# index-tts/index-tts

Measured on NVIDIA H100. Metric: speech_tokens_per_s, higher is better.
Workload: dtype bf16 GPT (bf16 weights/activations, fp32 accumulate, fp32 residual stream = the reference's use_bf16 autocast) + tail on wgmma with fp16 operands (.f16: DiT / WaveNet / BigVGAN-resblock GEMMs and the DiT flash attention; fp32 accumulate, fp32 softmax, fp32 residual streams and pointwise math) and tf

## Files before the change

index-tts_b200/csrc/gemm_tc.cu:

```cuda
#include "ops.h"
#include "ptx.cuh"
#include <cuda.h>
#include <cudaTypedefs.h>
#include <map>
#include <mutex>
#include <tuple>
#include <cstdlib>

namespace {

constexpr int BM = 128;
constexpr int BKB = 128;
constexpr int GEMM_THREADS = 160;

__device__ __forceinline__ float apply_act_tc(float v, int act) {
  switch (act) {
    case ACT_GELU_ERF: return 0.5f * v * (1.f + erff(v * 0.70710678118654752f));
    case ACT_SILU: return v / (1.f + __expf(-v));
    case ACT_MISH: {
      float sp = (v > 20.f) ? v : log1pf(__expf(v));
      return v * tanhf(sp);
    }
    case ACT_GELU_TANH: {
      float u = 0.7978845608028654f * (v + 0.044715f * v * v * v);
      return 0.5f * v * (1.f + tanhf(u));
    }
    case ACT_RELU: return v > 0.f ? v : 0.f;
    default: return v;
  }
}

struct TcParams {
  int M, N, K, taps, dil, pad, a_bcast, w_batched;
  int n_kchunks;
  const float* bias; int biasN; int act;
  const float* res; const float* rowscale; const float* colscale;
  int accum; float scale;
  float* out; long long out_batch_stride, out_off, out_valid; int ldo;
  int stages; int ring_bytes;
  int epi; __half* out16; const float* aux; int aux_stride;
};

constexpr int acc_tile_bytes(int BN) { return BM * (BN + 1) * 4; }

template <int BN, int EB>
__global__ void __launch_bounds__(GEMM_THREADS, 2)
gemm_tc_kernel(const __grid_constant__ CUtensorMap tmA, const __grid_constant__ CUtensorMap tmB,
               const TcParams p) {
  extern __shared__ __align__(1024) unsigned char smem_raw[];
  unsigned char* base = (unsigned char*)(((uintptr_t)smem_raw + 1023) & ~(uintptr_t)1023);
  constexpr int BK = BKB / EB;
  constexpr int A_BYTES = BM * BKB;
  constexpr int B_BYTES = BN * BKB;
  constexpr int STAGE_BYTES = A_BYTES + B_BYTES;
  constexpr int TP = BN + 1;
  uint64_t* full = (uint64_t*)(base + p.ring_bytes);
  uint64_t* empty = full + p.stages;

  const int warp = threadIdx.x >> 5, lane = threadIdx.x & 31;
  const int n0 = blockIdx.x * BN, m0 = blockIdx.y * BM, b = blockIdx.z;
  const int n_iters = p.taps * p.n_kchunks;

  if (threadIdx.x == 0) {
    for (int s = 0; s < p.stages; ++s) {
      ptx::mbar_init(&full[s], 1);
      ptx::mbar_init(&empty[s], 4);
    }
    ptx::fence_mbar_init();
  }
  __syncthreads();
  pdl_wait();
  pdl_trigger();

  if (warp == 4) {
    if (lane == 0) {
      ptx::prefetch_tensormap(&tmA);
      ptx::prefetch_tensormap(&tmB);
      for (int it = 0; it < n_iters; ++it) {
        const int s = it % p.stages;
        const uint32_t ph = (it / p.stages) & 1u;
        ptx::mbar_wait(&empty[s], ph ^ 1u);
        const int tap = it / p.n_kchunks, kc = it % p.n_kchunks;
        unsigned char* sa = base + (size_t)s * STAGE_BYTES;
        unsigned char* sb = sa + A_BYTES;
        ptx::mbar_arrive_expect_tx(&full[s], STAGE_BYTES);
        ptx::tma_load_3d(sa, &tmA, &full[s], kc * BK, m0 + tap * p.dil - p.pad, p.a_bcast ? 0 : b);
        ptx::tma_load_3d(sb, &tmB, &full[s], tap * p.K + kc * BK, n0, p.w_batched ? b : 0);
      }
    }
    return;
  }

  float acc0[BN / 2], acc1[BN / 2];
#pragma unroll
  for (int i = 0; i < BN / 2; ++i) { acc0[i] = 0.f; acc1[i] = 0.f; }
  for (int it = 0; it < n_iters; ++it) {
    const int s = it % p.stages;
    const uint32_t ph = (it / p.stages) & 1u;
    ptx::mbar_wait(&full[s], ph);
    const uint32_t sa = ptx::smem_u32(base + (size_t)s * STAGE_BYTES);
    const uint32_t sb = sa + A_BYTES;
    const uint64_t da = ptx::make_desc_sw128(sa), db = ptx::make_desc_sw128(sb);
    ptx::fence_regs(acc0);
    ptx::fence_regs(acc1);
    ptx::wgmma_fence();
#pragma unroll
    for (int k = 0; k < BKB / 32; ++k) {
      ptx::wgmma_ss<BN, EB>(acc0, da + (uint64_t)(2 * k), db + (uint64_t)(2 * k), 1u);
      ptx::wgmma_ss<BN, EB>(acc1, da + (uint64_t)(512 + 2 * k), db + (uint64_t)(2 * k), 1u);
    }
    ptx::wgmma_commit();
    ptx::wgmma_wait<1>();
    ptx::fence_regs(acc0);
    ptx::fence_regs(acc1);
    if (it > 0 && lane == 0) ptx::mbar_arrive(&empty[(it - 1) % p.stages]);
  }
  ptx::wgmma_wait<0>();
  ptx::fence_regs(acc0);
  ptx::fence_regs(acc1);

  ptx::named_bar_sync(1, 128);
  float* tile = (float*)base;
  {
    const int r0 = warp * 16 + (lane >> 2), c = 2 * (lane & 3);
#pragma unroll
    for (int j = 0; j < BN / 8; ++j) {
      float* t0 = tile + (size_t)r0 * TP + 8 * j + c;
      t0[0] = acc0[4 * j]; t0[1] = acc0[4 * j + 1];
      t0[8 * TP] = acc0[4 * j + 2]; t0[8 * TP + 1] = acc0[4 * j + 3];
      t0[64 * TP] = acc1[4 * j]; t0[64 * TP + 1] = acc1[4 * j + 1];
      t0[72 * TP] = acc1[4 * j + 2]; t0[72 * TP + 1] = acc1[4 * j + 3];
    }
  }
  ptx::named_bar_sync(1, 128);
  const int q = warp;
  const long long obs = p.out_batch_stride;
  const int biasN = p.biasN ? p.biasN : p.N;
  const int mrow0 = m0 + q * 32;
#pragma unroll 1
  for (int c0 = 0; c0 < BN; c0 += 32) {
    if (n0 + c0 >= p.N) break;
    const float* trow = tile + (size_t)(q * 32) * TP + c0;
    const int n = n0 + c0 + lane;
    if (p.epi != EPI_NONE) {
      const int row = mrow0 + lane;
      if (row < p.M) {
        const int nb = n0 + c0;
        float v[32];
#pragma unroll
        for (int j = 0; j < 32; ++j) v[j] = trow[lane * TP + j] + (p.bias ? __ldg(p.bias + nb + j) : 0.f);
        if (p.epi == EPI_ROPE) {
          const int HD = 64, Hh = p.aux_stride, HW = Hh * HD;
          const int which = nb / HW, hh = (nb % HW) / HD, d0 = nb % HD;
          __half* dst = p.out16 + (size_t)which * ((size_t)gridDim.z * Hh * p.M * HD) + (((size_t)b * Hh + hh) * (size_t)p.M + row) * HD + d0;
          uint32_t o[16];
          if (which < 2) {
            const float4* tab = (const float4*)(p.aux + ((size_t)row * (HD / 2) + (d0 >> 1)) * 2);
            const float sc = (which == 0) ? p.scale : 1.0f;
#pragma unroll
            for (int i = 0; i < 8; ++i) {
              const float4 t4 = __ldg(tab + i);
              const float a0 = v[4 * i], a1 = v[4 * i + 1], b0 = v[4 * i + 2], b1 = v[4 * i + 3];
              __half2 h0 = __floats2half2_rn((a0 * t4.x - a1 * t4.y) * sc, (a1 * t4.x + a0 * t4.y) * sc);
              __half2 h1 = __floats2half2_rn((b0 * t4.z - b1 * t4.w) * sc, (b1 * t4.z + b0 * t4.w) * sc);
              o[2 * i] = *(uint32_t*)&h0;
              o[2 * i + 1] = *(uint32_t*)&h1;
            }
          } else {
#pragma unroll
            for (int i = 0; i < 16; ++i) {
              __half2 h = __floats2half2_rn(v[2 * i], v[2 * i + 1]);
              o[i] = *(uint32_t*)&h;
            }
          }
#pragma unroll
          for (int i = 0; i < 4; ++i) ((uint4*)dst)[i] = make_uint4(o[4 * i], o[4 * i + 1], o[4 * i + 2], o[4 * i + 3]);
        } else {
          const int NH = p.N >> 1, j0 = nb >> 1;
          uint32_t o[8];
#pragma unroll
          for (int i = 0; i < 8; ++i) {
            float r0, r1;
            if (p.epi == EPI_SWIGLU) {
              r0 = __fdividef(v[4 * i], 1.f + __expf(-v[4 * i])) * v[4 * i + 1];
              r1 = __fdividef(v[4 * i + 2], 1.f + __expf(-v[4 * i + 2])) * v[4 * i + 3];
            } else {
              const float* ga = p.aux + (size_t)b * p.aux_stride + j0 + 2 * i;
              r0 = tanhf(v[4 * i] + __ldg(ga)) * __fdividef(1.f, 1.f + __expf(-(v[4 * i + 1] + __ldg(ga + NH))));
              r1 = tanhf(v[4 * i + 2] + __ldg(ga + 1)) * __fdividef(1.f, 1.f + __expf(-(v[4 * i + 3] + __ldg(ga + NH + 1))));
            }
            __half2 h = __floats2half2_rn(r0, r1);
            o[i] = *(uint32_t*)&h;
          }
          uint4* dst = (uint4*)(p.out16 + ((size_t)b * p.M + row) * NH + j0);
          dst[0] = make_uint4(o[0], o[1], o[2], o[3]);
          dst[1] = make_uint4(o[4], o[5], o[6], o[7]);
        }
      }
    } else if (n < p.N) {
      const float bv = p.bias ? __ldg(p.bias + (n % biasN)) : 0.f;
      const float cs = (p.colscale ? __ldg(p.colscale + n) : 1.f);
      const long long flat0 = p.out_off + (long long)mrow0 * p.ldo + n;
      const int rows = min(32, p.M - mrow0);
      const bool interior = rows == 32 && (p.out_off + (long long)mrow0 * p.ldo + n0 + c0) >= 0 &&
                            (p.out_off + (long long)(mrow0 + 31) * p.ldo + n0 + c0 + 31) < p.out_valid;
      float* op = p.out + (long long)b * obs + flat0;
      const float* rp = p.res ? p.res + (long long)b * obs + flat0 : nullptr;
      if (interior && p.act == ACT_NONE && !p.rowscale) {
        const float sc = p.scale;
        if (!rp && !p.accum) {
#pragma unroll 8
          for (int rr = 0; rr < 32; ++rr) op[(long long)rr * p.ldo] = (trow[rr * TP + lane] + bv) * cs * sc;
        } else {
          float addv[32];
#pragma unroll
          for (int rr = 0; rr < 32; ++rr) {
            float a = 0.f;
            if (rp) a = rp[(long long)rr * p.ldo];
            if (p.accum) a += op[(long long)rr * p.ldo];
            addv[rr] = a;
          }
#pragma unroll
          for (int rr = 0; rr < 32; ++rr)
            op[(long long)rr * p.ldo] = ((trow[rr * TP + lane] + bv) * cs + addv[rr]) * sc;
        }
      } else {
        for (int rr = 0; rr < rows; ++rr) {
          const long long flat = flat0 + (long long)rr * p.ldo;
          if (flat < 0 || flat >= p.out_valid) continue;
          float v = trow[rr * TP + lane] + bv;
          v = apply_act_tc(v, p.act) * cs;
          if (p.rowscale) v *= __ldg(p.rowscale + (long long)b * p.M + mrow0 + rr);
          if (rp) v += rp[(long long)rr * p.ldo];
          if (p.accum) v += op[(long long)rr * p.ldo];
          op[(long long)rr * p.ldo] = v * p.scale;
        }
      }
    }
  }
}

PFN_cuTensorMapEncodeTiled get_encode() {
  static PFN_cuTensorMapEncodeTiled fn = nullptr;
  if (!fn) {
    void* f = nullptr;
    cudaDriverEntryPointQueryResult qres;
    if (cudaGetDriverEntryPoint("cuTensorMapEncodeTiled", &f, cudaEnableDefault, &qres) != cudaSuccess || !f)
      throw IdxError(IDX_ERR_CUDA, "cuTensorMapEncodeTiled entry point not available");
    fn = (PFN_cuTensorMapEncodeTiled)f;
  }
  return fn;
}

using MapKey = std::tuple<const void*, long long, long long, long long, long long, int, int>;
std::map<MapKey, CUtensorMap>& map_cache() {
  static std::map<MapKey, CUtensorMap> c;
  return c;
}

CUtensorMap make_map(const void* ptr, int rank, const cuuint64_t* dims, const cuuint64_t* strides_bytes,
                     const cuuint32_t* box, bool half = false) {
  static const bool plain_f32 = getenv("IDX_TMA_F32") != nullptr;
  MapKey key(ptr, (long long)dims[0], (long long)dims[1], rank > 2 ? (long long)dims[2] : 0,
             (long long)strides_bytes[0] ^ ((rank > 2 ? (long long)strides_bytes[1] : 0) << 20), (int)box[1] | ((int)box[0] << 12), rank | (half ? 16 : 0));
  static std::mutex mu;
  std::lock_guard<std::mutex> lock(mu);
  auto& cache = map_cache();
  auto it = cache.find(key);
  if (it != cache.end()) return it->second;
  CUtensorMap m;
  cuuint32_t estr[3] = {1, 1, 1};
  CUresult r = get_encode()(&m, half ? CU_TENSOR_MAP_DATA_TYPE_FLOAT16 : (plain_f32 ? CU_TENSOR_MAP_DATA_TYPE_FLOAT32 : CU_TENSOR_MAP_DATA_TYPE_TFLOAT32),
                            (cuuint32_t)rank, const_cast<void*>(ptr), dims, strides_bytes, box, estr,
                            CU_TENSOR_MAP_INTERLEAVE_NONE, CU_TENSOR_MAP_SWIZZLE_128B,
                            CU_TENSOR_MAP_L2_PROMOTION_L2_128B, CU_TENSOR_MAP_FLOAT_OOB_FILL_NONE);
  if (r != CUDA_SUCCESS)
    throw IdxError(IDX_ERR_CUDA, "cuTensorMapEncodeTiled failed with code " + std::to_string((int)r));
  if (cache.size() > 20000) cache.clear();
  cache.emplace(key, m);
  return m;
}

template <int BN, int EB>
void launch_bn(idx_engine* e, const ConvGemm& g, const CUtensorMap& tmA, const CUtensorMap& tmB) {
  constexpr int BK = BKB / EB;
  TcParams p;
  p.M = g.M; p.N = g.N; p.K = g.K; p.taps = g.taps; p.dil = g.dil; p.pad = g.pad; p.a_bcast = g.a_bcast;
  p.w_batched = g.w_batch_stride != 0;
  p.n_kchunks = (g.K + BK - 1) / BK;
  p.bias = g.bias; p.biasN = g.biasN; p.act = g.act;
  p.res = g.res; p.rowscale = g.rowscale; p.colscale = g.colscale;
  p.accum = g.accum; p.scale = g.scale; p.out = g.out;
  p.ldo = g.ldo ? g.ldo : g.N;
  p.out_batch_stride = g.out_batch_stride ? g.out_batch_stride : (long long)g.M * g.N;
  p.out_off = g.out_off;
  p.out_valid = g.out_valid ? g.out_valid : (long long)g.M * p.ldo;
  p.epi = g.epi; p.out16 = g.out16; p.aux = g.aux; p.aux_stride = g.aux_stride;
  if (g.epi != EPI_NONE)
    IDX_CHECK(g.out16 && g.N % 32 == 0 && !g.res && !g.accum && g.act == ACT_NONE && (g.epi == EPI_SWIGLU || g.aux), IDX_ERR_ARG,
              "conv_gemm: bad fused-epilogue arguments");
  constexpr int STAGE = BM * BKB + BN * BKB;
  const int n_iters = p.taps * p.n_kchunks;
  static const int occ = getenv("IDX_GEMM_OCC") ? atoi(getenv("IDX_GEMM_OCC")) : 2;
  int stages = ((occ == 1 ? 208 : 104) * 1024) / STAGE;
  if (stages > 8) stages = 8;
  if (stages > n_iters) stages = n_iters < 2 ? 2 : n_iters;
  p.stages = stages;
  p.ring_bytes = ((stages * STAGE > acc_tile_bytes(BN) ? stages * STAGE : acc_tile_bytes(BN)) + 1023) & ~1023;
  const size_t smem = (size_t)p.ring_bytes + 1024 + 2 * stages * 8;
  const unsigned bit = (BN == 32 ? 1u : (BN == 64 ? 2u : 4u)) << (EB == 2 ? 8 : 0);
  if (!(e->attr_done & bit)) {
    IDX_CUDA(cudaFuncSetAttribute(gemm_tc_kernel<BN, EB>, cudaFuncAttributeMaxDynamicSharedMemorySize, 220 * 1024));
    e->attr_done |= bit;
  }
  dim3 grid((g.N + BN - 1) / BN, (g.M + BM - 1) / BM, g.B);
  launch_pdl(e, gemm_tc_kernel<BN, EB>, grid, dim3(GEMM_THREADS), smem, tmA, tmB, p);
  e->launches++;
}


constexpr int FA_Q = 128, FA_K = 128, FA_D = 64;
constexpr int FA_THREADS = 288;
__device__ __forceinline__ float ex2_approx(float x) {
  float y;
  asm("ex2.approx.ftz.f32 %0, %1;" : "=f"(y) : "f"(x));
  return y;
}
__device__ __forceinline__ uint32_t pack_half2(float lo, float hi) {
  __half2 h = __floats2half2_rn(lo, hi);
  return *(uint32_t*)&h;
}
struct FaParams {
  int T, H; float* out; __half* out16; const int4* tiles;
  const int* lens; const float* qe; int rel_l, rel_r;
};
template <int SEL>
__device__ __forceinline__ void fa_add_relkey(float (&S)[FA_K / 2], const float* qr, int r, int k0, int t4, int L, int R) {
  if (k0 + FA_K - 1 - r <= -L || k0 - r >= R) {
    const float c = qr[k0 - r >= R ? L + R : 0];
#pragma unroll
    for (int c8 = 0; c8 < FA_K / 8; ++c8) { S[4 * c8 + SEL] += c; S[4 * c8 + SEL + 1] += c; }
  } else {
#pragma unroll
    for (int c8 = 0; c8 < FA_K / 8; ++c8) {
      const int d = k0 + 8 * c8 + 2 * t4 - r;
      S[4 * c8 + SEL] += qr[min(max(d, -L), R) + L];
      S[4 * c8 + SEL + 1] += qr[min(max(d + 1, -L), R) + L];
    }
  }
}
constexpr int FA_QE = 80;
// ... 265 lines not shown
```

index-tts_b200/csrc/nn_ops.cu:

```cuda
#include "ops.h"
#include <cuda_bf16.h>
#include <cstdlib>

namespace {

__device__ __forceinline__ float warp_sum(float v) {
#pragma unroll
  for (int o = 16; o > 0; o >>= 1) v += __shfl_xor_sync(0xffffffffu, v, o);
  return v;
}

__device__ __forceinline__ void put(float* __restrict__ y, __half* __restrict__ y16, long long i, float v) {
  if (y) y[i] = v;
  if (y16) y16[i] = __float2half_rn(v);
}

template <int MODE>
__global__ void rownorm_kernel(const float* __restrict__ x, float* __restrict__ y, long long rows, int T,
                               int C, const float* __restrict__ w, const float* __restrict__ b, float eps,
                               const float* __restrict__ m0, const float* __restrict__ m1, int mod_stride,
                               __half* __restrict__ y16) {
  pdl_wait();
  const long long row = (long long)blockIdx.x * (blockDim.x >> 5) + (threadIdx.x >> 5);
  const int lane = threadIdx.x & 31;
// ... 90 lines not shown
  const int t = blockIdx.y;
  const int c = blockIdx.x * blockDim.x + threadIdx.x;
  const int id = ids[t];
  const bool ok = id >= 0 && id < nrows;
  if (!ok && c == 0) atomicCAS(bad, 0, t + 1);
  if (c < C) out[(long long)t * C + c] = ok ? table[(long long)id * C + c] : 0.f;
}

__global__ void swiglu_kernel(const float* __restrict__ ab, float* __restrict__ y, long long rows, int N, __half* __restrict__ y16) {
  pdl_wait();
  const long long i = (long long)blockIdx.x * blockDim.x + threadIdx.x;
  if (i >= rows * N) return;
  const long long r = i / N;
  const int c = (int)(i % N);
  const float a = ab[r * 2 * N + c], b = ab[r * 2 * N + N + c];
  put(y, y16, i, a / (1.f + expf(-a)) * b);
}

__global__ void wn_gate_kernel(const float* __restrict__ xin, const float* __restrict__ g, int g_stride,
                               float* __restrict__ y, int T, int N, __half* __restrict__ y16) {
  pdl_wait();
  const int bi = blockIdx.z;
  const long long i = (long long)blockIdx.x * blockDim.x + threadIdx.x;
  if (i >= (long long)T * N) return;
  const long long t = i / N;
  const int c = (int)(i % N);
  const float* xr = xin + ((long long)bi * T + t) * 2 * N;
  const float a = xr[c] + g[(long long)bi * g_stride + c];
  const float s = xr[N + c] + g[(long long)bi * g_stride + N + c];
  put(y, y16, ((long long)bi * T + t) * N + c, tanhf(a) * (1.f / (1.f + expf(-s))));
}

__global__ void copy_cols_kernel(const float* __restrict__ src, int lds, float* __restrict__ dst, int ldo,
                                 int col0, long long rows, int C, __half* __restrict__ dst16) {
  pdl_wait();
  const long long i = (long long)blockIdx.x * blockDim.x + threadIdx.x;
  if (i >= rows * C) return;
  const long long r = i / C;
  const int c = (int)(i % C);
  put(dst, dst16, r * ldo + col0 + c, src[r * lds + c]);
}
__global__ void bcast_cols_kernel(const float* __restrict__ vec, float* __restrict__ dst, int ldo, int col0,
                                  int T, int C) {
  const int bi = blockIdx.z;
  const long long i = (long long)blockIdx.x * blockDim.x + threadIdx.x;
  if (i >= (long long)T * C) return;
  const long long t = i / C;
  const int c = (int)(i % C);
  dst[((long long)bi * T + t) * ldo + col0 + c] = vec[(long long)bi * C + c];
}
__global__ void silu_kernel(float* x, long long n) {
  const long long i = (long long)blockIdx.x * blockDim.x + threadIdx.x;
  if (i < n) { const float v = x[i]; x[i] = v / (1.f + expf(-v)); }
}
__device__ __forceinline__ int reflect_src(int i, int T, int left, int right) {
  const int Tr = max(T, max(left, right) + 1);
  int t = i - left;
  if (t < 0) t = -t;
  if (t >= Tr) t = 2 * (Tr - 1) - t;
  return t < T ? t : -1;
}
__global__ void reflect_pad_kernel(const float* __restrict__ x, float* __restrict__ y, int T, int C, int left, int right,
                                   int Tout, __half* __restrict__ y16) {
  pdl_wait();
  const int bi = blockIdx.z;
  const int c = blockIdx.x * blockDim.x + threadIdx.x;
  if (c >= C) return;
  for (int i = blockIdx.y; i < Tout; i += gridDim.y) {
    const int t = reflect_src(i, T, left, right);
    put(y, y16, ((long long)bi * Tout + i) * C + c, t >= 0 ? x[((long long)bi * T + t) * C + c] : 0.f);
  }
}
__device__ __forceinline__ int segment_of(const int* __restrict__ off, int n, int r, int gap) {
  int lo = 0, hi = n - 1;
  while (lo < hi) {
    const int mid = (lo + hi + 1) >> 1;
    if (off[mid] + mid * gap <= r) lo = mid; else hi = mid - 1;
  }
  return lo;
}
__global__ void reflect_pad_seg_kernel(const float* __restrict__ x, __half* __restrict__ y16, int T, int C, int left, int gap,
                                       int Tout, const int* __restrict__ off, int n) {
  pdl_wait();
  const int bi = blockIdx.z;
  const int c = blockIdx.x * blockDim.x + threadIdx.x;
  if (c >= C) return;
  for (int i = blockIdx.y; i < Tout; i += gridDim.y) {
    const int u = segment_of(off, n, i, gap);
    const int t0 = off[u], Tu = off[u + 1] - t0;
    const int t = reflect_src(i - t0 - u * gap, Tu, left, gap - left);
    y16[((long long)bi * Tout + i) * C + c] = __float2half_rn(t >= 0 ? x[((long long)bi * T + t0 + t) * C + c] : 0.f);
  }
}
__global__ void compact_seg_kernel(const __half* __restrict__ x, __half* __restrict__ y, int T, int Mg, int C, int gap,
                                   const int* __restrict__ off, int n) {
  pdl_wait();
  const int bi = blockIdx.z;
  const int c = (blockIdx.x * blockDim.x + threadIdx.x) * 8;
  if (c >= C) return;
  for (int r = blockIdx.y; r < T; r += gridDim.y) {
    const int u = segment_of(off, n, r, 0);
    *(uint4*)(y + ((long long)bi * T + r) * C + c) = *(const uint4*)(x + ((long long)bi * Mg + r + u * gap) * C + c);
  }
}
__global__ void cfg_euler_rows_kernel(float* x, const float* vc, const float* vu, float dt, float rate, int T, int C,
                                      const unsigned char* __restrict__ zero_rows) {
  pdl_wait();
  const long long i = (long long)blockIdx.x * blockDim.x + threadIdx.x;
  if (i >= (long long)T * C) return;
  const int t = (int)(i / C);
  const float d = (1.0f + rate) * vc[i] - rate * vu[i];
  x[i] = zero_rows[t] ? 0.f : x[i] + dt * d;
}
// ... 598 lines not shown
```

index-tts_b200/csrc/ops.h:

```cpp
#pragma once
#include "engine.h"
#include <cuda_fp16.h>
#include <cstdlib>
#include <string>
#include <utility>
#include <vector>

enum { EPI_NONE = 0, EPI_SWIGLU = 1, EPI_WNGATE = 2, EPI_ROPE = 3 };
enum { ACT_NONE = 0, ACT_GELU_ERF = 1, ACT_SILU = 2, ACT_MISH = 3, ACT_GELU_TANH = 4, ACT_RELU = 5 };

struct ConvGemm {
  const float* A = nullptr;
  int B = 1, Tin = 0, K = 0;
  long long a_batch_stride = 0;
  int a_bcast = 0;
  int lda = 0;
  const float* W = nullptr;
  const float* Wk = nullptr;
  const __half* A16 = nullptr;
  const __half* Wk16 = nullptr;
  int epi = 0;
  __half* out16 = nullptr;
  const float* aux = nullptr;
  int aux_stride = 0;
  long long w_batch_stride = 0;
  int ldw = 0;
  int taps = 1, dil = 1, pad = 0, reflect = 0;
  int M = 0;
  int N = 0;
  const float* bias = nullptr;
  int biasN = 0;
  int act = ACT_NONE;
  const float* res = nullptr;
  const float* rowscale = nullptr;
  const float* colscale = nullptr;
  int accum = 0;
  float scale = 1.f;
  float* out = nullptr;
  long long out_batch_stride = 0;
  long long out_off = 0;
  long long out_valid = 0;
  int ldo = 0;
};

void conv_gemm(idx_engine* e, const ConvGemm& g);
inline int gemm_default_backend(const idx_engine* e) { return e->gemm_backend; }

void transpose_bct_to_btc(idx_engine* e, const float* in, float* out, int B, int C, int T);
void transpose_btc_to_bct(idx_engine* e, const float* in, float* out, int B, int T, int C);

#ifdef __CUDACC__
__device__ __forceinline__ void pdl_wait() { asm volatile("griddepcontrol.wait;" ::: "memory"); }
__device__ __forceinline__ void pdl_trigger() { asm volatile("griddepcontrol.launch_dependents;" ::: "memory"); }
template <typename... KArgs, typename... Args>
inline void launch_pdl(idx_engine* e, void (*kernel)(KArgs...), dim3 grid, dim3 block, size_t smem, Args&&... args) {
  static const bool off = getenv("IDX_PDL") && atoi(getenv("IDX_PDL")) == 0;
  cudaLaunchConfig_t cfg = {};
  cfg.gridDim = grid; cfg.blockDim = block; cfg.dynamicSmemBytes = smem; cfg.stream = e->stream;
  cudaLaunchAttribute attr[1];
  attr[0].id = cudaLaunchAttributeProgrammaticStreamSerialization;
  attr[0].val.programmaticStreamSerializationAllowed = 1;
  cfg.attrs = attr; cfg.numAttrs = off ? 0 : 1;
  IDX_CUDA(cudaLaunchKernelEx(&cfg, kernel, std::forward<Args>(args)...));
}
#endif

void layernorm(idx_engine* e, const float* x, float* y, int B, int T, int C, const float* w,
               const float* b, float eps, const float* scale, const float* shift, int mod_stride, __half* y16 = nullptr);
void rmsnorm_adaln(idx_engine* e, const float* x, float* y, int B, int T, int C, const float* nw,
                   const float* mw, const float* mb, int mod_stride, float eps, __half* y16 = nullptr);
void groupnorm1_mish(idx_engine* e, const float* x, float* y, int B, int T, int C, const float* w,
                     const float* b, float eps);
void dwconv1d(idx_engine* e, const float* x, float* y, int B, int T, int C, const float* w,
              const float* b, int k);
void nearest_interp(idx_engine* e, const float* x, float* y, int B, int Tin, int Tout, int C);
void embedding_rows(idx_engine* e, const float* table, const int* ids, float* out, int n, int C, int nrows);
void swiglu(idx_engine* e, const float* ab, float* y, long long rows, int N, __half* y16 = nullptr);
void wn_gate(idx_engine* e, const float* xin, const float* g, int g_stride, float* y, int B, int T, int N, __half* y16 = nullptr);
void copy_cols(idx_engine* e, const float* src, int lds, float* dst, int ldo, int col0, long long rows, int C, __half* dst16 = nullptr);
void bcast_cols(idx_engine* e, const float* vec, float* dst, int ldo, int col0, int B, int T, int C);
void silu_inplace(idx_engine* e, float* x, long long n);
void rope_table(idx_engine* e, float* tab, int T, int hd);
void attention_rope(idx_engine* e, const float* qkv, float* out, int B, int T, int H, const float* rope,
                    const int* lens, __half* out16 = nullptr);
void cfg_euler(idx_engine* e, float* x, const float* v_cond, const float* v_uncond, float dt, float rate,
               int T, int C, int P);
void fill_zero(idx_engine* e, float* x, long long n);
struct DebugOverrides {
  idx_engine* e;
  ~DebugOverrides() { e->force_backend = 0; e->force_tile_n = 0; }
};
void reflect_pad_rows(idx_engine* e, const float* x, float* y, int B, int T, int C, int left, int right, __half* y16 = nullptr);

struct PackedW {
  float* wsimt = nullptr;
  float* wk = nullptr;
  __half* wk16 = nullptr;
  const float* bias = nullptr;
  int N = 0, K = 0, taps = 1, dil = 1;
};
struct WeightPool {
  std::vector<void*> owned;
  float* alloc(size_t n);
  void release();
};
PackedW pack_linear(idx_engine* e, WeightPool& pool, const std::string& name, int row0 = 0, int rows = -1,
// ... 39 lines not shown
```

index-tts_b200/csrc/s2mel.cu:

```cuda
#include "stages.h"
#include <algorithm>
#include <cmath>
#include <cstring>

namespace {

__global__ void timestep_embed_kernel(const float* t, const float* freqs, float* out, int half) {
  const int k = blockIdx.x, i = threadIdx.x;
  if (i >= half) return;
  const float a = 1000.f * t[k] * freqs[i];
  out[(long long)k * 2 * half + i] = cosf(a);
  out[(long long)k * 2 * half + half + i] = sinf(a);
}

__global__ void gamma_residual_kernel(const float* y, const float* gamma, float* x, long long rows, int C) {
  const long long i = (long long)blockIdx.x * blockDim.x + threadIdx.x;
  if (i >= rows * C) return;
  x[i] += gamma[i % C] * y[i];
}

}

struct AdaLN {
  const float* norm_w = nullptr;
  int mod_off = 0;
};

struct S2melState {
  idx_s2mel_config cfg;
  idx_codec_config ccfg;
  bool has_s2mel = false, has_codec = false;
  WeightPool pool;
  int inter = 0;
  std::vector<PackedW> wqkv, wo, w13, w2, skip_in;
  std::vector<AdaLN> attn_norm, ffn_norm;
  AdaLN final_norm;
  PackedW mod_stack;
  PackedW cond_proj, merge_x, merge_rest, skip_linear, conv1, res_proj, fl_linear, conv2, fl_mod;
  PackedW te_mlp0, te_mlp2, te2_mlp0, te2_mlp2, wn_cond;
  const float *te_freqs = nullptr, *te2_freqs = nullptr;
  std::vector<PackedW> wn_in, wn_res, wn_skip;
  std::vector<__half*> w13_i16, wn_in_i16;
  std::vector<float*> wn_in_bias_i;
  int mod_width = 0;
  PackedW lr_in_proj, lr_out;
  std::vector<PackedW> lr_conv;
  std::vector<const float*> lr_gn_w, lr_gn_b;
  PackedW cd_out_proj, cd_embed, cd_head, cd_up;
  const float* cd_codebook = nullptr;
  const float *cd_norm_w = nullptr, *cd_norm_b = nullptr, *cd_fnorm_w = nullptr, *cd_fnorm_b = nullptr;
  struct CNX { const float *dw_w, *dw_b, *n_w, *n_b, *gamma; PackedW pw1, pw2; };
  std::vector<CNX> cnx;
  double ms_codec = 0, ms_lr = 0, ms_cfm = 0;
  cudaEvent_t ev0 = nullptr, ev1 = nullptr;
};

void s2mel_destroy(S2melState* s) {
  if (!s) return;
  s->pool.release();
  if (s->ev0) cudaEventDestroy(s->ev0);
  if (s->ev1) cudaEventDestroy(s->ev1);
  delete s;
}

static S2melState* state(idx_engine* e) {
  if (!e->s2mel) {
    e->s2mel = new S2melState();
    IDX_CUDA(cudaEventCreate(&e->s2mel->ev0));
    IDX_CUDA(cudaEventCreate(&e->s2mel->ev1));
  }
  return e->s2mel;
}

static PackedW pack_stacked(idx_engine* e, WeightPool& pool, const std::vector<std::string>& names, float** bias_out) {
  int K = -1, N = 0;
  for (auto& n : names) {
    const DevTensor& w = e->W(n + ".weight");
    IDX_CHECK(w.shape.size() >= 2, IDX_ERR_ARG, n + ": bad shape");
    if (K < 0) K = (int)w.shape[1];
    IDX_CHECK((int)w.shape[1] == K, IDX_ERR_ARG, n + ": K mismatch in stacked pack");
    N += (int)w.shape[0];
  }
  float* cat = nullptr;
  IDX_CUDA(cudaMalloc((void**)&cat, (size_t)N * K * 4));
  float* bias = pool.alloc(N);
  IDX_CUDA(cudaMemsetAsync(bias, 0, (size_t)N * 4, e->stream));
  int r = 0;
  for (auto& n : names) {
    const DevTensor& w = e->W(n + ".weight");
    const int rows = (int)w.shape[0];
    IDX_CUDA(cudaMemcpyAsync(cat + (size_t)r * K, w.d, (size_t)rows * K * 4, cudaMemcpyDeviceToDevice, e->stream));
    if (e->has(n + ".bias"))
      IDX_CUDA(cudaMemcpyAsync(bias + r, e->W(n + ".bias").d, (size_t)rows * 4, cudaMemcpyDeviceToDevice, e->stream));
    r += rows;
// ... 28 lines not shown
  s->attn_norm.clear(); s->ffn_norm.clear();
  for (int l = 0; l < Dn; ++l) {
    const std::string p = E + "transformer.layers." + std::to_string(l) + ".";
    s->wqkv.push_back(pack_linear(e, s->pool, p + "attention.wqkv"));
    s->wo.push_back(pack_linear(e, s->pool, p + "attention.wo"));
    s->w13.push_back(pack_stacked(e, s->pool, {p + "feed_forward.w1", p + "feed_forward.w3"}, nullptr));
    s->w13.back().bias = nullptr;
    s->w2.push_back(pack_linear(e, s->pool, p + "feed_forward.w2"));
    s->skip_in.push_back(pack_linear(e, s->pool, p + "skip_in_linear"));
    AdaLN a; a.norm_w = e->Wf(p + "attention_norm.norm.weight"); a.mod_off = (int)mods.size() * 2 * H;
    mods.push_back(p + "attention_norm.project_layer");
    AdaLN f; f.norm_w = e->Wf(p + "ffn_norm.norm.weight"); f.mod_off = (int)mods.size() * 2 * H;
    mods.push_back(p + "ffn_norm.project_layer");
    s->attn_norm.push_back(a);
    s->ffn_norm.push_back(f);
  }
  s->final_norm.norm_w = e->Wf(E + "transformer.norm.norm.weight");
  s->final_norm.mod_off = (int)mods.size() * 2 * H;
  mods.push_back(E + "transformer.norm.project_layer");
  s->mod_stack = pack_stacked(e, s->pool, mods, nullptr);
  s->mod_width = (int)mods.size() * 2 * H;
  s->cond_proj = pack_linear(e, s->pool, E + "cond_projection");
  {
    const DevTensor& w = e->W(E + "cond_x_merge_linear.weight");
    const int Kall = (int)w.shape[1];
    IDX_CHECK(Kall == H + 2 * C + cfg->style_dim, IDX_ERR_ARG, "cond_x_merge_linear shape");
    std::vector<float> h((size_t)H * Kall);
    IDX_CUDA(cudaMemcpy(h.data(), w.d, h.size() * 4, cudaMemcpyDeviceToHost));
    std::vector<float> hx((size_t)H * C), hr((size_t)H * (Kall - C));
    for (int r = 0; r < H; ++r) {
      memcpy(&hx[(size_t)r * C], &h[(size_t)r * Kall], (size_t)C * 4);
      memcpy(&hr[(size_t)r * (Kall - C)], &h[(size_t)r * Kall + C], (size_t)(Kall - C) * 4);
    }
    int64_t shx[2] = {H, C}, shr[2] = {H, Kall - C};
    IDX_CHECK(idx_load_weight(e, "__merge_x.weight", hx.data(), IDX_F32, 2, shx) == 0, IDX_ERR_ARG, e->err);
    IDX_CHECK(idx_load_weight(e, "__merge_rest.weight", hr.data(), IDX_F32, 2, shr) == 0, IDX_ERR_ARG, e->err);
    s->merge_x = pack_linear(e, s->pool, "__merge_x", 0, -1, false);
    s->merge_rest = pack_linear(e, s->pool, "__merge_rest", 0, -1, false);
    s->merge_rest.bias = e->Wf(E + "cond_x_merge_linear.bias");
  }
  s->skip_linear = pack_linear(e, s->pool, E + "skip_linear");
  s->conv1 = pack_linear(e, s->pool, E + "conv1");
  s->res_proj = pack_linear(e, s->pool, E + "res_projection");
  s->fl_linear = pack_linear(e, s->pool, E + "final_layer.linear");
  s->fl_mod = pack_linear(e, s->pool, E + "final_layer.adaLN_modulation.1");
  s->conv2 = pack_linear(e, s->pool, E + "conv2");
  s->te_mlp0 = pack_linear(e, s->pool, E + "t_embedder.mlp.0");
  s->te_mlp2 = pack_linear(e, s->pool, E + "t_embedder.mlp.2");
  s->te2_mlp0 = pack_linear(e, s->pool, E + "t_embedder2.mlp.0");
  s->te2_mlp2 = pack_linear(e, s->pool, E + "t_embedder2.mlp.2");
  s->te_freqs = e->Wf(E + "t_embedder.freqs");
  s->te2_freqs = e->Wf(E + "t_embedder2.freqs");
  s->wn_cond = pack_linear(e, s->pool, E + "wavenet.cond_layer.conv.conv");
  s->wn_in.clear(); s->wn_res.clear(); s->wn_skip.clear();
  for (int i = 0; i < NL; ++i) {
    const std::string wi = E + "wavenet.in_layers." + std::to_string(i) + ".conv.conv";
    const std::string wr = E + "wavenet.res_skip_layers." + std::to_string(i) + ".conv.conv";
    s->wn_in.push_back(pack_conv1d(e, s->pool, wi, 1));
    IDX_CHECK(s->wn_in.back().taps == cfg->wn_kernel, IDX_ERR_ARG, "wavenet kernel size");
    if (i < NL - 1) {
      s->wn_res.push_back(pack_linear(e, s->pool, wr, 0, WH));
      s->wn_skip.push_back(pack_linear(e, s->pool, wr, WH, WH));
    } else {
      s->wn_res.push_back(PackedW());
      s->wn_skip.push_back(pack_linear(e, s->pool, wr, 0, WH));
    }
  }
  const std::string R = "s2mel.length_regulator.";
  s->lr_in_proj = pack_linear(e, s->pool, R + "content_in_proj");
  s->lr_conv.clear(); s->lr_gn_w.clear(); s->lr_gn_b.clear();
  for (int i = 0; i < cfg->lr_convs; ++i) {
    s->lr_conv.push_back(pack_conv1d(e, s->pool, R + "model." + std::to_string(3 * i), 1));
    s->lr_gn_w.push_back(e->Wf(R + "model." + std::to_string(3 * i + 1) + ".weight"));
    s->lr_gn_b.push_back(e->Wf(R + "model." + std::to_string(3 * i + 1) + ".bias"));
  }
  s->lr_out = pack_linear(e, s->pool, R + "model." + std::to_string(3 * cfg->lr_convs));
  IDX_CUDA(cudaStreamSynchronize(e->stream));
  for (auto* v : {&s->wqkv, &s->wo, &s->w13, &s->w2, &s->skip_in, &s->wn_in, &s->wn_res, &s->wn_skip})
    for (auto& w : *v) pack_half(e, s->pool, w);
  for (auto* w : {&s->skip_linear, &s->conv1, &s->res_proj, &s->fl_linear, &s->conv2}) pack_half(e, s->pool, *w);
  s->w13_i16.clear(); s->wn_in_i16.clear(); s->wn_in_bias_i.clear();
  for (auto& w : s->w13) s->w13_i16.push_back(pack_half_interleaved(e, s->pool, w, nullptr));
  for (auto& w : s->wn_in) {
    float* bi = nullptr;
    s->wn_in_i16.push_back(pack_half_interleaved(e, s->pool, w, &bi));
    s->wn_in_bias_i.push_back(bi);
  }
  s->has_s2mel = true;
  IDX_API_END(e)
}

extern "C" int idx_codec_init(idx_engine* e, const idx_codec_config* cfg) {
  IDX_API_BEGIN
  IDX_CHECK(e && cfg, IDX_ERR_ARG, "null argument");
  IDX_CUDA(cudaSetDevice(e->device));
  S2melState* s = state(e);
  s->ccfg = *cfg;
  const std::string Q = "codec.quantizer.quantizers.0.", D = "codec.decoder.0.";
  s->cd_codebook = e->Wf(Q + "codebook.weight");
  s->cd_out_proj = pack_linear(e, s->pool, Q + "out_project");
  s->cd_embed = pack_conv1d(e, s->pool, D + "embed", 1);
  s->cd_norm_w = e->Wf(D + "norm.weight"); s->cd_norm_b = e->Wf(D + "norm.bias");
  s->cd_fnorm_w = e->Wf(D + "final_layer_norm.weight"); s->cd_fnorm_b = e->Wf(D + "final_layer_norm.bias");
  s->cnx.clear();
  for (int l = 0; l < cfg->vocos_num_layers; ++l) {
    const std::string p = D + "convnext." + std::to_string(l) + ".";
    S2melState::CNX c;
    c.dw_w = e->Wf(p + "dwconv.weight"); c.dw_b = e->Wf(p + "dwconv.bias");
    c.n_w = e->Wf(p + "norm.weight"); c.n_b = e->Wf(p + "norm.bias");
    c.gamma = e->Wf(p + "gamma");
    c.pw1 = pack_linear(e, s->pool, p + "pwconv1");
    c.pw2 = pack_linear(e, s->pool, p + "pwconv2");
    s->cnx.push_back(c);
  }
  s->cd_head = pack_linear(e, s->pool, "codec.decoder.1");
  s->cd_up = pack_conv1d(e, s->pool, "codec.up", 1);
  IDX_CUDA(cudaStreamSynchronize(e->stream));
  s->has_codec = true;
  IDX_API_END(e)
}

void codec_decode_dev(idx_engine* e, S2melState* s, const int* d_codes, int n, float* d_out) {
  const idx_codec_config& c = s->ccfg;
  const int Hs = c.hidden_size, Vd = c.vocos_dim, Vi = c.vocos_intermediate_dim;
  float* emb = e->arena.get<float>((size_t)n * c.codebook_dim);
  float* q = e->arena.get<float>((size_t)n * Hs);
  float* x = e->arena.get<float>((size_t)n * Vd);
  float* y = e->arena.get<float>((size_t)n * Vd);
  float* hbuf = e->arena.get<float>((size_t)n * Vi);
  float* up = e->arena.get<float>((size_t)2 * n * Hs);
  embedding_rows(e, s->cd_codebook, d_codes, emb, n, c.codebook_dim, c.codebook_size);
// ... 69 lines not shown
  for (int l = 0; l < Dn; ++l) {
    if (l > Dn / 2) {
      float* sk = skips[--nskip];
      copy_cols(e, h, H, hf ? nullptr : b.cat, 2 * H, 0, (long long)Bn * T, H, b.cat16);
      copy_cols(e, sk, H, hf ? nullptr : b.cat, 2 * H, H, (long long)Bn * T, H, b.cat16);
      float* hn = b.h[8 + (l & 1)];
      conv_gemm(e, G(s->skip_in[l], b.cat, b.cat16, Bn, T, hn));
      h = hn;
    }
    rmsnorm_adaln(e, h, hf ? nullptr : b.a, Bn, T, H, s->attn_norm[l].norm_w, mod + s->attn_norm[l].mod_off,
                  mod + s->attn_norm[l].mod_off + H, 0, 1e-5f, b.a16);
    if (hf && fused) {
      ConvGemm g = gemm_of16(s->wqkv[l], b.a16, Bn, T, nullptr);
      g.epi = EPI_ROPE; g.out16 = b.qkv16; g.aux = b.rope; g.aux_stride = nh;
      g.scale = flash_attention_q_scale();
      conv_gemm(e, g);
      const size_t one = (size_t)Bn * nh * T * 64;
      if (b.sg) flash_attention_wgmma_varlen(e, b.qkv16, b.qkv16 + one, b.qkv16 + 2 * one, nullptr, b.att16, Bn, nh, *b.sg);
      else flash_attention_split(e, b.qkv16, b.qkv16 + one, b.qkv16 + 2 * one, nullptr, b.att16, Bn, T, nh);
    } else {
      conv_gemm(e, G(s->wqkv[l], b.a, b.a16, Bn, T, b.qkv));
      attention_rope(e, b.qkv, hf ? nullptr : b.att, Bn, T, nh, b.rope, b.lens, b.att16);
    }
    float* hout = (l < Dn / 2) ? b.h[1 + l] : b.h[10 + (l & 1)];
    {
      ConvGemm g = G(s->wo[l], b.att, b.att16, Bn, T, hout);
      g.res = h;
      conv_gemm(e, g);
    }
    rmsnorm_adaln(e, hout, hf ? nullptr : b.a, Bn, T, H, s->ffn_norm[l].norm_w, mod + s->ffn_norm[l].mod_off,
                  mod + s->ffn_norm[l].mod_off + H, 0, 1e-5f, b.a16);
    if (hf && fused) {
      ConvGemm g = gemm_of16(s->w13[l], b.a16, Bn, T, nullptr);
      g.Wk16 = s->w13_i16[l]; g.bias = nullptr; g.epi = EPI_SWIGLU; g.out16 = b.ffh16;
      conv_gemm(e, g);
    } else {
      conv_gemm(e, G(s->w13[l], b.a, b.a16, Bn, T, b.ff));
      swiglu(e, b.ff, hf ? nullptr : b.qkv, (long long)Bn * T, s->inter, b.ffh16);
    }
    {
      ConvGemm g = G(s->w2[l], b.qkv, b.ffh16, Bn, T, hout);
      g.res = hout;
      conv_gemm(e, g);
    }
    h = hout;
    if (l < Dn / 2) skips[nskip++] = h;
  }
  rmsnorm_adaln(e, h, b.a, Bn, T, H, s->final_norm.norm_w, mod + s->final_norm.mod_off,
                mod + s->final_norm.mod_off + H, 0, 1e-5f);
  copy_cols(e, b.a, H, hf ? nullptr : b.cat, H + C, 0, (long long)Bn * T, H, b.cat16);
  for (int bi = 0; bi < Bn; ++bi)
    copy_cols(e, x_bcast ? x_t : x_t + (size_t)bi * T * C, C, hf ? nullptr : b.cat + (size_t)bi * T * (H + C), H + C, H, T, C,
              hf ? b.cat16 + (size_t)bi * T * (H + C) : nullptr);
  conv_gemm(e, G(s->skip_linear, b.cat, b.cat16, Bn, T, b.xres));
  if (hf) to_half(e, b.xres, b.xres16, (long long)Bn * T * H);
  conv_gemm(e, G(s->conv1, b.xres, b.xres16, Bn, T, b.wy));
  fill_zero(e, b.wout, (long long)Bn * T * WH);
  for (int i = 0; i < NL; ++i) {
    const int kk = s->wn_in[i].taps, pl = (kk - 1) - (kk - 1) / 2, pr = (kk - 1) / 2;
    if (b.sg) {
      const int gap = kk - 1, ng = b.sg->n();
      reflect_pad_segments(e, b.wy, b.wpad16, Bn, WH, pl, pr, *b.sg);
      ConvGemm gi = gemm_of16(s->wn_in[i], b.wpad16, Bn, T + ng * gap, nullptr);
      gi.pad = 0; gi.M = T + (ng - 1) * gap;
      gi.Wk16 = s->wn_in_i16[i]; gi.bias = s->wn_in_bias_i[i];
      gi.epi = EPI_WNGATE; gi.out16 = b.wacts16g; gi.aux = wncond + (size_t)i * 2 * WH; gi.aux_stride = 0;
      conv_gemm(e, gi);
      compact_segments16(e, b.wacts16g, b.wacts16, Bn, WH, gap, *b.sg);
    } else {
      reflect_pad_rows(e, b.wy, hf ? nullptr : b.wpad, Bn, T, WH, pl, pr, b.wpad16);
      ConvGemm gi = G(s->wn_in[i], b.wpad, b.wpad16, Bn, T + kk - 1, b.wxin);
      gi.pad = 0; gi.M = T;
      if (hf && fused) {
        gi.Wk16 = s->wn_in_i16[i]; gi.bias = s->wn_in_bias_i[i]; gi.out = nullptr;
        gi.epi = EPI_WNGATE; gi.out16 = b.wacts16; gi.aux = wncond + (size_t)i * 2 * WH; gi.aux_stride = 0;
        conv_gemm(e, gi);
      } else {
        conv_gemm(e, gi);
        wn_gate(e, b.wxin, wncond + (size_t)i * 2 * WH, 0, hf ? nullptr : b.wacts, Bn, T, WH, b.wacts16);
      }
    }
    if (i < NL - 1) {
      ConvGemm gr = G(s->wn_res[i], b.wacts, b.wacts16, Bn, T, b.wy);
      gr.res = b.wy;
      conv_gemm(e, gr);
    }
    ConvGemm gs = G(s->wn_skip[i], b.wacts, b.wacts16, Bn, T, b.wout);
    gs.accum = 1;
    conv_gemm(e, gs);
  }
  {
    ConvGemm g = G(s->res_proj, b.xres, b.xres16, Bn, T, b.wout);
    g.accum = 1;
    conv_gemm(e, g);
  }
  layernorm(e, b.wout, hf ? nullptr : b.z, Bn, T, WH, nullptr, nullptr, 1e-6f, flmod + WH, flmod, 0, b.z16);
  conv_gemm(e, G(s->fl_linear, b.z, b.z16, Bn, T, b.wy));
  if (hf) to_half(e, b.wy, b.wy16, (long long)Bn * T * WH);
  conv_gemm(e, G(s->conv2, b.wy, b.wy16, Bn, T, b.v));
}

static void alloc_dit(idx_engine* e, S2melState* s, DitBuffers& b, int Bn, int T, const Segments* sg = nullptr) {
  const idx_s2mel_config& c = s->cfg;
  const int H = c.hidden, WH = c.wn_hidden, C = c.in_channels;
  const size_t bt = (size_t)Bn * T;
  if (sg && sg->n() == 1) sg = nullptr;
  for (int i = 0; i < 12; ++i) b.h[i] = e->arena.get<float>(bt * H);
  b.a = e->arena.get<float>(bt * H);
  b.qkv = e->arena.get<float>(bt * (size_t)std::max(3 * H, s->inter));
  b.att = e->arena.get<float>(bt * H);
  b.ff = e->arena.get<float>(bt * 2 * s->inter);
  b.cat = e->arena.get<float>(bt * 2 * H);
  b.xres = e->arena.get<float>(bt * H);
  b.wy = e->arena.get<float>(bt * WH);
  const size_t padT = (size_t)T + 8 * (sg ? sg->n() : 1);
  b.wpad = e->arena.get<float>((size_t)Bn * padT * WH);
  b.wxin = e->arena.get<float>(bt * 2 * WH);
  b.wacts = e->arena.get<float>(bt * WH);
  b.wout = e->arena.get<float>(bt * WH);
  b.z = e->arena.get<float>(bt * WH);
  b.v = e->arena.get<float>(bt * C);
  b.rope = e->arena.get<float>((size_t)T * 64);
  b.lens = nullptr;
  if (tail_half(e) && !attn_unfused() && H % 8 == 0 && WH % 8 == 0 && (H + C) % 8 == 0 && s->inter % 8 == 0) {
    auto hb = [&](size_t n) { return (__half*)e->arena.alloc(n * sizeof(__half) + 16); };
    b.a16 = hb(bt * H); b.att16 = hb(bt * H); b.ffh16 = hb(bt * s->inter); b.cat16 = hb(bt * 2 * H);
    b.xres16 = hb(bt * H); b.wpad16 = hb((size_t)Bn * padT * WH); b.wacts16 = hb(bt * WH); b.z16 = hb(bt * WH);
    b.wy16 = hb(bt * WH);
    b.qkv16 = hb(3 * bt * H);
  }
  b.sg = sg;
  if (sg) {
    IDX_CHECK(b.a16 && tail_fused() && fa_wgmma_on(), IDX_ERR_STATE, "packed solve outside the fp16 fused tail mode");
    b.wacts16g = (__half*)e->arena.alloc((size_t)Bn * padT * WH * sizeof(__half) + 16);
    rope_table_segments(e, b.rope, *sg, 64);
  } else {
    rope_table(e, b.rope, T, 64);
  }
}
static size_t dit_arena_bytes(const S2melState* s, int Bn, int T, int nseg) {
  const idx_s2mel_config& c = s->cfg;
  const size_t bt = (size_t)Bn * T, pad = (size_t)Bn * (T + 8 * (size_t)nseg) * c.wn_hidden;
  const size_t Tp = (size_t)((T + 3) & ~3);
  const size_t attn = nseg > 1 ? 0 : 4 * (size_t)Bn * c.heads * (3 * (size_t)T * 64 + 64 * Tp + (attn_unfused() ? (size_t)T * Tp : 0)) + 8 * 256;
  const size_t half_bytes = 2 * (bt * c.hidden * 8 + bt * s->inter + bt * c.wn_hidden * 3 + (nseg > 1 ? 2 : 1) * pad) + 16 * 512;
  return attn + half_bytes + 4 * (bt * c.hidden * 20 + bt * 3 * s->inter + bt * c.wn_hidden * 6 + pad + bt * c.in_channels +
                                  (size_t)T * 64) + 64 * 256;
}

struct TimeTables { float *mod, *wncond, *flmod; };
static TimeTables time_tables(idx_engine* e, S2melState* s, const float* d_t, int nt) {
// ... 272 lines not shown
```

Baseline: 1014.

## Fuse fp16 output, reflect padding, and WaveNet res/skip GEMMs into GEMM epilogue

Adds an EPI_OUT16 epilogue mode to the tensor-core GEMM. It writes the fp16 copy of the output, and optionally the reflect-padded fp16 buffer, directly, which removes separate to_half and reflect_pad_rows kernels in the DiT/WaveNet tail. It also merges each WaveNet layer's res and skip 1x1 convs into one GEMM. That GEMM splits its columns: the low half goes to the residual (with fp16 copy), the high half accumulates into the skip output, which removes the fill_zero and one GEMM launch per layer. The cost is extra branching and scattered 2-byte stores in the epilogue, plus per-warp reflect-pad writes that rely on the tile holding the source row.

New measurement: 1022 (median of 6 runs). Within noise of the previous version (+0.8%).

```diff
diff --git a/index-tts_b200/csrc/gemm_tc.cu b/index-tts_b200/csrc/gemm_tc.cu
--- a/index-tts_b200/csrc/gemm_tc.cu
+++ b/index-tts_b200/csrc/gemm_tc.cu
@@ -39,6 +39,7 @@
   float* out; long long out_batch_stride, out_off, out_valid; int ldo;
   int stages; int ring_bytes;
   int epi; __half* out16; const float* aux; int aux_stride;
+  int n16, pad16_l, pad16_r; float* out2; int accum2;
 };
 
 constexpr int acc_tile_bytes(int BN) { return BM * (BN + 1) * 4; }
@@ -142,7 +143,7 @@
     if (n0 + c0 >= p.N) break;
     const float* trow = tile + (size_t)(q * 32) * TP + c0;
     const int n = n0 + c0 + lane;
-    if (p.epi != EPI_NONE) {
+    if (p.epi != EPI_NONE && p.epi != EPI_OUT16) {
       const int row = mrow0 + lane;
       if (row < p.M) {
         const int nb = n0 + c0;
@@ -198,42 +199,68 @@
         }
       }
     } else if (n < p.N) {
+      const bool hi = p.epi == EPI_OUT16 && n0 + c0 >= p.n16;
+      const int ldo = hi ? p.N - p.n16 : p.ldo;
+      const long long ob = hi ? (long long)p.M * ldo : obs, off = hi ? -(long long)p.n16 : p.out_off;
+      const long long valid = hi ? (long long)p.M * ldo : p.out_valid;
+      float* const obase = hi ? p.out2 : p.out;
+      const int accum = hi ? p.accum2 : p.accum;
+      __half* const o16 = (p.epi == EPI_OUT16 && !hi && p.out16)
+          ? p.out16 + ((long long)b * (p.M + p.pad16_l + p.pad16_r) + p.pad16_l) * p.n16 + n : nullptr;
       const float bv = p.bias ? __ldg(p.bias + (n % biasN)) : 0.f;
       const float cs = (p.colscale ? __ldg(p.colscale + n) : 1.f);
-      const long long flat0 = p.out_off + (long long)mrow0 * p.ldo + n;
+      const long long flat0 = off + (long long)mrow0 * ldo + n;
       const int rows = min(32, p.M - mrow0);
-      const bool interior = rows == 32 && (p.out_off + (long long)mrow0 * p.ldo + n0 + c0) >= 0 &&
-                            (p.out_off + (long long)(mrow0 + 31) * p.ldo + n0 + c0 + 31) < p.out_valid;
-      float* op = p.out + (long long)b * obs + flat0;
-      const float* rp = p.res ? p.res + (long long)b * obs + flat0 : nullptr;
+      const bool interior = rows == 32 && (off + (long long)mrow0 * ldo + n0 + c0) >= 0 &&
+                            (off + (long long)(mrow0 + 31) * ldo + n0 + c0 + 31) < valid;
+      float* op = obase ? obase + (long long)b * ob + flat0 : nullptr;
+      const float* rp = (p.res && !hi) ? p.res + (long long)b * ob + flat0 : nullptr;
       if (interior && p.act == ACT_NONE && !p.rowscale) {
         const float sc = p.scale;
-        if (!rp && !p.accum) {
+        if (!rp && !accum && !hi) {
 #pragma unroll 8
-          for (int rr = 0; rr < 32; ++rr) op[(long long)rr * p.ldo] = (trow[rr * TP + lane] + bv) * cs * sc;
+          for (int rr = 0; rr < 32; ++rr) {
+            const float v = (trow[rr * TP + lane] + bv) * cs * sc;
+            if (op) op[(long long)rr * ldo] = v;
+            if (o16) o16[(long long)(mrow0 + rr) * p.n16] = __float2half_rn(v);
+          }
         } else {
           float addv[32];
 #pragma unroll
           for (int rr = 0; rr < 32; ++rr) {
             float a = 0.f;
-            if (rp) a = rp[(long long)rr * p.ldo];
-            if (p.accum) a += op[(long long)rr * p.ldo];
+            if (rp) a = rp[(long long)rr * ldo];
+            if (accum) a += op[(long long)rr * ldo];
             addv[rr] = a;
           }
 #pragma unroll
-          for (int rr = 0; rr < 32; ++rr)
-            op[(long long)rr * p.ldo] = ((trow[rr * TP + lane] + bv) * cs + addv[rr]) * sc;
+          for (int rr = 0; rr < 32; ++rr) {
+            const float v = ((trow[rr * TP + lane] + bv) * cs + addv[rr]) * sc;
+            op[(long long)rr * ldo] = v;
+            if (o16) o16[(long long)(mrow0 + rr) * p.n16] = __float2half_rn(v);
+          }
         }
       } else {
         for (int rr = 0; rr < rows; ++rr) {
-          const long long flat = flat0 + (long long)rr * p.ldo;
-          if (flat < 0 || flat >= p.out_valid) continue;
+          const long long flat = flat0 + (long long)rr * ldo;
+          if (flat < 0 || flat >= valid) continue;
           float v = trow[rr * TP + lane] + bv;
           v = apply_act_tc(v, p.act) * cs;
           if (p.rowscale) v *= __ldg(p.rowscale + (long long)b * p.M + mrow0 + rr);
-          if (rp) v += rp[(long long)rr * p.ldo];
-          if (p.accum) v += op[(long long)rr * p.ldo];
-          op[(long long)rr * p.ldo] = v * p.scale;
+          if (rp) v += rp[(long long)rr * ldo];
+          if (accum || hi) v += accum ? op[(long long)rr * ldo] : 0.f;
+          v *= p.scale;
+          if (op) op[(long long)rr * ldo] = v;
+          if (o16) o16[(long long)(mrow0 + rr) * p.n16] = __float2half_rn(v);
+        }
+      }
+      if (o16 && rows > 0) {
+        for (int i = 0; i < p.pad16_l + p.pad16_r; ++i) {
+          const int fr = i < p.pad16_l ? i : p.M + i;
+          const int t = reflect_src(fr, p.M, p.pad16_l, p.pad16_r);
+          __half* dst = o16 + (long long)(fr - p.pad16_l) * p.n16;
+          if (t >= mrow0 && t < mrow0 + rows) *dst = o16[(long long)t * p.n16];
+          else if (t < 0 && mrow0 == 0) *dst = __float2half_rn(0.f);
         }
       }
     }
@@ -296,7 +323,15 @@
   p.out_off = g.out_off;
   p.out_valid = g.out_valid ? g.out_valid : (long long)g.M * p.ldo;
   p.epi = g.epi; p.out16 = g.out16; p.aux = g.aux; p.aux_stride = g.aux_stride;
-  if (g.epi != EPI_NONE)
+  p.n16 = g.n16 ? g.n16 : g.N; p.pad16_l = g.pad16_l; p.pad16_r = g.pad16_r; p.out2 = g.out2; p.accum2 = g.accum2;
+  if (g.epi == EPI_OUT16) {
+    IDX_CHECK(p.n16 % 32 == 0 && p.n16 <= g.N && (p.n16 == g.N || g.out2) && (g.out || (g.out16 && !g.res && !g.accum)) &&
+              g.act == ACT_NONE && !g.rowscale && !g.colscale && !g.out_off && !g.out_valid && (!g.ldo || g.ldo == p.n16) &&
+              !g.out_batch_stride && g.pad16_l >= 0 && g.pad16_r >= 0, IDX_ERR_ARG, "conv_gemm: bad EPI_OUT16 arguments");
+    p.ldo = p.n16;
+    p.out_batch_stride = (long long)g.M * p.n16;
+    p.out_valid = p.out_batch_stride;
+  } else if (g.epi != EPI_NONE)
     IDX_CHECK(g.out16 && g.N % 32 == 0 && !g.res && !g.accum && g.act == ACT_NONE && (g.epi == EPI_SWIGLU || g.aux), IDX_ERR_ARG,
               "conv_gemm: bad fused-epilogue arguments");
   constexpr int STAGE = BM * BKB + BN * BKB;
diff --git a/index-tts_b200/csrc/nn_ops.cu b/index-tts_b200/csrc/nn_ops.cu
--- a/index-tts_b200/csrc/nn_ops.cu
+++ b/index-tts_b200/csrc/nn_ops.cu
@@ -166,13 +166,6 @@
 __global__ void silu_kernel(float* x, long long n) {
   const long long i = (long long)blockIdx.x * blockDim.x + threadIdx.x;
   if (i < n) { const float v = x[i]; x[i] = v / (1.f + expf(-v)); }
-}
-__device__ __forceinline__ int reflect_src(int i, int T, int left, int right) {
-  const int Tr = max(T, max(left, right) + 1);
-  int t = i - left;
-  if (t < 0) t = -t;
-  if (t >= Tr) t = 2 * (Tr - 1) - t;
-  return t < T ? t : -1;
 }
 __global__ void reflect_pad_kernel(const float* __restrict__ x, float* __restrict__ y, int T, int C, int left, int right,
                                    int Tout, __half* __restrict__ y16) {
diff --git a/index-tts_b200/csrc/ops.h b/index-tts_b200/csrc/ops.h
--- a/index-tts_b200/csrc/ops.h
+++ b/index-tts_b200/csrc/ops.h
@@ -6,7 +6,7 @@
 #include <utility>
 #include <vector>
 
-enum { EPI_NONE = 0, EPI_SWIGLU = 1, EPI_WNGATE = 2, EPI_ROPE = 3 };
+enum { EPI_NONE = 0, EPI_SWIGLU = 1, EPI_WNGATE = 2, EPI_ROPE = 3, EPI_OUT16 = 4 };
 enum { ACT_NONE = 0, ACT_GELU_ERF = 1, ACT_SILU = 2, ACT_MISH = 3, ACT_GELU_TANH = 4, ACT_RELU = 5 };
 
 struct ConvGemm {
@@ -21,6 +21,10 @@
   const __half* Wk16 = nullptr;
   int epi = 0;
   __half* out16 = nullptr;
+  int n16 = 0;
+  int pad16_l = 0, pad16_r = 0;
+  float* out2 = nullptr;
+  int accum2 = 0;
   const float* aux = nullptr;
   int aux_stride = 0;
   long long w_batch_stride = 0;
@@ -52,6 +56,13 @@
 #ifdef __CUDACC__
 __device__ __forceinline__ void pdl_wait() { asm volatile("griddepcontrol.wait;" ::: "memory"); }
 __device__ __forceinline__ void pdl_trigger() { asm volatile("griddepcontrol.launch_dependents;" ::: "memory"); }
+__device__ __forceinline__ int reflect_src(int i, int T, int left, int right) {
+  const int Tr = max(T, max(left, right) + 1);
+  int t = i - left;
+  if (t < 0) t = -t;
+  if (t >= Tr) t = 2 * (Tr - 1) - t;
+  return t < T ? t : -1;
+}
 template <typename... KArgs, typename... Args>
 inline void launch_pdl(idx_engine* e, void (*kernel)(KArgs...), dim3 grid, dim3 block, size_t smem, Args&&... args) {
   static const bool off = getenv("IDX_PDL") && atoi(getenv("IDX_PDL")) == 0;
diff --git a/index-tts_b200/csrc/s2mel.cu b/index-tts_b200/csrc/s2mel.cu
--- a/index-tts_b200/csrc/s2mel.cu
+++ b/index-tts_b200/csrc/s2mel.cu
@@ -40,6 +40,7 @@
   PackedW te_mlp0, te_mlp2, te2_mlp0, te2_mlp2, wn_cond;
   const float *te_freqs = nullptr, *te2_freqs = nullptr;
   std::vector<PackedW> wn_in, wn_res, wn_skip;
+  std::vector<PackedW> wn_rs;
   std::vector<__half*> w13_i16, wn_in_i16;
   std::vector<float*> wn_in_bias_i;
   int mod_width = 0;
@@ -174,7 +175,7 @@
   s->te_freqs = e->Wf(E + "t_embedder.freqs");
   s->te2_freqs = e->Wf(E + "t_embedder2.freqs");
   s->wn_cond = pack_linear(e, s->pool, E + "wavenet.cond_layer.conv.conv");
-  s->wn_in.clear(); s->wn_res.clear(); s->wn_skip.clear();
+  s->wn_in.clear(); s->wn_res.clear(); s->wn_skip.clear(); s->wn_rs.clear();
   for (int i = 0; i < NL; ++i) {
     const std::string wi = E + "wavenet.in_layers." + std::to_string(i) + ".conv.conv";
     const std::string wr = E + "wavenet.res_skip_layers." + std::to_string(i) + ".conv.conv";
@@ -183,6 +184,7 @@
     if (i < NL - 1) {
       s->wn_res.push_back(pack_linear(e, s->pool, wr, 0, WH));
       s->wn_skip.push_back(pack_linear(e, s->pool, wr, WH, WH));
+      s->wn_rs.push_back(pack_linear(e, s->pool, wr, 0, 2 * WH));
     } else {
       s->wn_res.push_back(PackedW());
       s->wn_skip.push_back(pack_linear(e, s->pool, wr, 0, WH));
@@ -198,7 +200,7 @@
   }
   s->lr_out = pack_linear(e, s->pool, R + "model." + std::to_string(3 * cfg->lr_convs));
   IDX_CUDA(cudaStreamSynchronize(e->stream));
-  for (auto* v : {&s->wqkv, &s->wo, &s->w13, &s->w2, &s->skip_in, &s->wn_in, &s->wn_res, &s->wn_skip})
+  for (auto* v : {&s->wqkv, &s->wo, &s->w13, &s->w2, &s->skip_in, &s->wn_in, &s->wn_res, &s->wn_skip, &s->wn_rs})
     for (auto& w : *v) pack_half(e, s->pool, w);
   for (auto* w : {&s->skip_linear, &s->conv1, &s->res_proj, &s->fl_linear, &s->conv2}) pack_half(e, s->pool, *w);
   s->w13_i16.clear(); s->wn_in_i16.clear(); s->wn_in_bias_i.clear();
@@ -374,12 +376,22 @@
   for (int bi = 0; bi < Bn; ++bi)
     copy_cols(e, x_bcast ? x_t : x_t + (size_t)bi * T * C, C, hf ? nullptr : b.cat + (size_t)bi * T * (H + C), H + C, H, T, C,
               hf ? b.cat16 + (size_t)bi * T * (H + C) : nullptr);
-  conv_gemm(e, G(s->skip_linear, b.cat, b.cat16, Bn, T, b.xres));
-  if (hf) to_half(e, b.xres, b.xres16, (long long)Bn * T * H);
-  conv_gemm(e, G(s->conv1, b.xres, b.xres16, Bn, T, b.wy));
-  fill_zero(e, b.wout, (long long)Bn * T * WH);
+  const bool f16epi = hf && fused;
+  const bool padfused = f16epi && !b.sg;
+  const int kk = c.wn_kernel, pl = (kk - 1) - (kk - 1) / 2, pr = (kk - 1) / 2;
+  {
+    ConvGemm g = G(s->skip_linear, b.cat, b.cat16, Bn, T, b.xres);
+    if (f16epi) { g.epi = EPI_OUT16; g.out = nullptr; g.out16 = b.xres16; }
+    conv_gemm(e, g);
+    if (hf && !f16epi) to_half(e, b.xres, b.xres16, (long long)Bn * T * H);
+  }
+  {
+    ConvGemm g = G(s->conv1, b.xres, b.xres16, Bn, T, b.wy);
+    if (padfused) { g.epi = EPI_OUT16; g.out16 = b.wpad16; g.pad16_l = pl; g.pad16_r = pr; }
+    conv_gemm(e, g);
+  }
+  if (!f16epi || NL == 1) fill_zero(e, b.wout, (long long)Bn * T * WH);
   for (int i = 0; i < NL; ++i) {
-    const int kk = s->wn_in[i].taps, pl = (kk - 1) - (kk - 1) / 2, pr = (kk - 1) / 2;
     if (b.sg) {
       const int gap = kk - 1, ng = b.sg->n();
       reflect_pad_segments(e, b.wy, b.wpad16, Bn, WH, pl, pr, *b.sg);
@@ -390,7 +402,7 @@
       conv_gemm(e, gi);
       compact_segments16(e, b.wacts16g, b.wacts16, Bn, WH, gap, *b.sg);
     } else {
-      reflect_pad_rows(e, b.wy, hf ? nullptr : b.wpad, Bn, T, WH, pl, pr, b.wpad16);
+      if (!padfused) reflect_pad_rows(e, b.wy, hf ? nullptr : b.wpad, Bn, T, WH, pl, pr, b.wpad16);
       ConvGemm gi = G(s->wn_in[i], b.wpad, b.wpad16, Bn, T + kk - 1, b.wxin);
       gi.pad = 0; gi.M = T;
       if (hf && fused) {
@@ -402,6 +414,13 @@
         wn_gate(e, b.wxin, wncond + (size_t)i * 2 * WH, 0, hf ? nullptr : b.wacts, Bn, T, WH, b.wacts16);
       }
     }
+    if (f16epi && i < NL - 1) {
+      ConvGemm g = gemm_of16(s->wn_rs[i], b.wacts16, Bn, T, b.wy);
+      g.res = b.wy; g.epi = EPI_OUT16; g.n16 = WH; g.out2 = b.wout; g.accum2 = i > 0;
+      if (padfused) { g.out16 = b.wpad16; g.pad16_l = pl; g.pad16_r = pr; }
+      conv_gemm(e, g);
+      continue;
+    }
     if (i < NL - 1) {
       ConvGemm gr = G(s->wn_res[i], b.wacts, b.wacts16, Bn, T, b.wy);
       gr.res = b.wy;
@@ -417,8 +436,12 @@
     conv_gemm(e, g);
   }
   layernorm(e, b.wout, hf ? nullptr : b.z, Bn, T, WH, nullptr, nullptr, 1e-6f, flmod + WH, flmod, 0, b.z16);
-  conv_gemm(e, G(s->fl_linear, b.z, b.z16, Bn, T, b.wy));
-  if (hf) to_half(e, b.wy, b.wy16, (long long)Bn * T * WH);
+  {
+    ConvGemm g = G(s->fl_linear, b.z, b.z16, Bn, T, b.wy);
+    if (f16epi) { g.epi = EPI_OUT16; g.out = nullptr; g.out16 = b.wy16; }
+    conv_gemm(e, g);
+    if (hf && !f16epi) to_half(e, b.wy, b.wy16, (long long)Bn * T * WH);
+  }
   conv_gemm(e, G(s->conv2, b.wy, b.wy16, Bn, T, b.v));
 }
 
```
